# W-Ted/F3D-Gaus

Hardware: AMD Instinct MI355X
Metric: rendered views/sec at 256x256 (N Gaussians, K cams) (higher is better)
Workload: dtype f32; 1 GPU; C2: 1 image/GPU, 196608 Gaussians (sigma0=0.01), 120-view orbit @256x256, GOF forward raster only; timed region = render + 8-bit RGB frames copied to pinned host memory; compositing arithmetic: fast = error-free float32 pairs for the float64 island + hardware exp/rcp/rsq; every channel within 1e-4 of the oracle (RGB <= 3e-7), EXCEPT that the distortion channel (values 1e-7..1e-5 from cancelling fl; gaussians=196608, views=120, resolution=256, tile_cull=1, views_per_call=120, render_mode=fast, channels=all, parallelism=single GPU

## Files before the change

### f3d-gaus_amd/csrc/f3dg_binning.hip

```cpp
#include "f3dg_common.h"

namespace {

typedef unsigned long long u64;
typedef unsigned int u32;

__global__ void __launch_bounds__(F3DG_BLOCK)
scan_reduce_kernel(const u32* __restrict__ in, u64 n, u32* __restrict__ block_sums)
{
    __shared__ u32 wsum[F3DG_BLOCK / 64];
    const u64 base = (u64)blockIdx.x * F3DG_SCAN_CHUNK;
    u32 s = 0;
#pragma unroll
    for (int i = 0; i < F3DG_SCAN_ITEMS; i++) {
        const u64 k = base + (u64)i * F3DG_BLOCK + threadIdx.x;
        if (k < n) s += in[k];
    }
#pragma unroll
    for (int off = 32; off > 0; off >>= 1) s += __shfl_down(s, off, 64);
    if ((threadIdx.x & 63) == 0) wsum[threadIdx.x >> 6] = s;
    __syncthreads();
    if (threadIdx.x == 0) block_sums[blockIdx.x] = wsum[0] + wsum[1] + wsum[2] + wsum[3];
}

__global__ void __launch_bounds__(1024)
scan_blocksums_kernel(u32* __restrict__ block_sums, u32 nblocks, F3dgHeader* __restrict__ hdr)
{
    __shared__ u32 wtot[16];
    __shared__ u32 carry_s;
    __shared__ u64 carry64_s, wtot64[16];
    if (threadIdx.x == 0) { carry_s = 0; carry64_s = 0; }
    __syncthreads();
    const int lane = threadIdx.x & 63, wave = threadIdx.x >> 6;
    for (u32 start = 0; start < nblocks; start += 1024) {
        const u32 i = start + threadIdx.x;
        const u32 v = i < nblocks ? block_sums[i] : 0;
        u32 x = v;
#pragma unroll
        for (int off = 1; off < 64; off <<= 1) {
            const u32 y = __shfl_up(x, off, 64);
            if (lane >= off) x += y;
        }
        if (lane == 63) wtot[wave] = x;
        unsigned long long v64 = v;
#pragma unroll
        for (int off = 32; off > 0; off >>= 1) v64 += __shfl_down(v64, off, 64);
        if (lane == 0) wtot64[wave] = v64;
        __syncthreads();
        u32 wave_off = 0;
        for (int w = 0; w < wave; w++) wave_off += wtot[w];
        const u32 carry = carry_s;
        if (i < nblocks) block_sums[i] = carry + wave_off + x - v;
        __syncthreads();
        if (threadIdx.x == 1023) {
            carry_s = carry + wave_off + x;
            u64 t = 0;
            for (int w = 0; w < 16; w++) t += wtot64[w];
            carry64_s += t;
        }
        __syncthreads();
    }
    if (hdr && threadIdx.x == 0) {
        const u64 total = carry64_s;
        hdr->num_rendered = total > 0xFFFFFFFFull ? 0xFFFFFFFFu : (u32)total;
        hdr->overflow = total > (u64)hdr->capacity ? 1u : 0u;
    }
}

__global__ void __launch_bounds__(F3DG_BLOCK)
scan_apply_kernel(const u32* in, u32* out , u64 n, const u32* __restrict__ block_sums,
                  int exclusive)
{
    __shared__ u32 wtot[F3DG_BLOCK / 64];
    const u64 base = (u64)blockIdx.x * F3DG_SCAN_CHUNK + (u64)threadIdx.x * F3DG_SCAN_ITEMS;
    u32 v[F3DG_SCAN_ITEMS];
    u32 s = 0;
    if (base + F3DG_SCAN_ITEMS <= n) {
#pragma unroll
        for (int i = 0; i < F3DG_SCAN_ITEMS / 4; i++) {
            const uint4 w = reinterpret_cast<const uint4*>(in + base)[i];
            v[4 * i] = w.x; v[4 * i + 1] = w.y; v[4 * i + 2] = w.z; v[4 * i + 3] = w.w;
        }
    } else {
#pragma unroll
        for (int i = 0; i < F3DG_SCAN_ITEMS; i++) v[i] = (base + i < n) ? in[base + i] : 0;
    }
#pragma unroll
    for (int i = 0; i < F3DG_SCAN_ITEMS; i++) s += v[i];
    const int lane = threadIdx.x & 63, wave = threadIdx.x >> 6;
    u32 x = s;
#pragma unroll
    for (int off = 1; off < 64; off <<= 1) {
        const u32 y = __shfl_up(x, off, 64);
        if (lane >= off) x += y;
    }
    if (lane == 63) wtot[wave] = x;
    __syncthreads();
    u32 run = block_sums[blockIdx.x] + x - s;
    for (int w = 0; w < wave; w++) run += wtot[w];
    u32 o[F3DG_SCAN_ITEMS];
#pragma unroll
    for (int i = 0; i < F3DG_SCAN_ITEMS; i++) {
        const u32 before = run;
        run += v[i];
        o[i] = exclusive ? before : run;
    }
    if (base + F3DG_SCAN_ITEMS <= n) {
#pragma unroll
        for (int i = 0; i < F3DG_SCAN_ITEMS / 4; i++)
            reinterpret_cast<uint4*>(out + base)[i] = make_uint4(o[4 * i], o[4 * i + 1], o[4 * i + 2], o[4 * i + 3]);
    } else {
#pragma unroll
        for (int i = 0; i < F3DG_SCAN_ITEMS; i++)
            if (base + i < n) out[base + i] = o[i];
    }
}


struct SegChunk {
    u64 seg_base;
    u64 obase;
    u32 n;
    u32 cps;
    u32 c;
    u32 seg;
};

struct SegTable {
    const u32* vstart;
    const u32* bglob;
    const u32* xprefix;
    u32 xstride;
    u32 V;
};

struct ShiftDigit {
    int shift;
    u32 mask = 255u;
    __device__ __forceinline__ u32 operator()(u32 k) const { return (k >> shift) & mask; }
};
struct CompactDigit {
    u32 kbase;
    __device__ __forceinline__ u32 operator()(u32 k) const { const u32 d = (k - kbase) >> 16; return d < 255u ? d : 255u; }
};

template <typename K, typename DIGIT, bool MINMAX = false>
__device__ __forceinline__ void hist_chunk(const K* __restrict__ keys, const SegChunk& ck, const DIGIT digit, u32* __restrict__ hist,
                                           u32 (*h)[256], u32* __restrict__ minmax = nullptr)
{
    u32 kmin = 0xFFFFFFFFu, kmax = 0u;
#pragma unroll
    for (int w = 0; w < F3DG_BLOCK / 64; w++) h[w][threadIdx.x] = 0;
    __syncthreads();
    u32* hw = h[threadIdx.x >> 6];
    constexpr int VEC = 16 / (int)sizeof(K);
    typedef K __attribute__((ext_vector_type(VEC))) KV;
    const u64 base = (u64)ck.c * F3DG_SORT_CHUNK;
    const u64 g0 = ck.seg_base + base;
    const u64 g1 = ck.seg_base + ((u64)ck.n - base < (u64)F3DG_SORT_CHUNK ? (u64)ck.n : base + F3DG_SORT_CHUNK);
    for (u64 a = (g0 & ~(u64)(VEC - 1)) + (u64)threadIdx.x * VEC; a < g1; a += (u64)F3DG_BLOCK * VEC) {
        const KV w = *reinterpret_cast<const KV*>(keys + a);
#pragma unroll
        for (int q = 0; q < VEC; q++) {
            if (a + q >= g0 && a + q < g1) {
                const u32 key = (u32)w[q];
                atomicAdd(&hw[digit(key)], 1u);
                if (MINMAX && key != 0xFFFFFFFFu) { kmin = key < kmin ? key : kmin; kmax = key > kmax ? key : kmax; }
            }
        }
    }
    __shared__ u32 wmm[2][F3DG_BLOCK / 64];
    if (MINMAX) {
#pragma unroll
        for (int off = 32; off > 0; off >>= 1) {
            const u32 a = __shfl_down(kmin, off, 64), b = __shfl_down(kmax, off, 64);
            kmin = a < kmin ? a : kmin; kmax = b > kmax ? b : kmax;
        }
        if ((threadIdx.x & 63) == 0) { wmm[0][threadIdx.x >> 6] = kmin; wmm[1][threadIdx.x >> 6] = kmax; }
    }
    __syncthreads();
    if (MINMAX && threadIdx.x == 0) {
        u32 a = wmm[0][0], b = wmm[1][0];
#pragma unroll
        for (int w = 1; w < F3DG_BLOCK / 64; w++) { a = wmm[0][w] < a ? wmm[0][w] : a; b = wmm[1][w] > b ? wmm[1][w] : b; }
        minmax[0] = a; minmax[1] = b;
    }
    hist[ck.obase + (u64)threadIdx.x * ck.cps + ck.c] = h[0][threadIdx.x] + h[1][threadIdx.x] + h[2][threadIdx.x] + h[3][threadIdx.x];
}

struct ScatterShared {
    u32 cnt[F3DG_BLOCK / 64][256];
    u32 lbase[256];
    u32 gdelta[256];
    u32 wtot[F3DG_BLOCK / 64];
    u32 sval[F3DG_SORT_CHUNK];
};

template <typename K, bool IOTA, typename DIGIT>
__device__ __forceinline__ void scatter_chunk(const K* __restrict__ keys_in, const u32* __restrict__ vals_in, K* __restrict__ keys_out,
                                              u32* __restrict__ vals_out, const SegChunk& ck, const DIGIT digit,
                                              const u32* __restrict__ offsets , ScatterShared& sh, K* skey)
{
    const u32 n = ck.n;
    const u64 block_base = (u64)ck.c * F3DG_SORT_CHUNK;
    const u32 in_block = (u32)((n - block_base) < (u64)F3DG_SORT_CHUNK ? (n - block_base) : (u64)F3DG_SORT_CHUNK);
    const int lane = threadIdx.x & 63, wave = threadIdx.x >> 6;
#pragma unroll
    for (int w = 0; w < F3DG_BLOCK / 64; w++) sh.cnt[w][threadIdx.x] = 0;
    __syncthreads();

    const u64 wave_base = block_base + (u64)wave * (64 * F3DG_SORT_ITEMS);
    u32 key[F3DG_SORT_ITEMS];
    u32 val[F3DG_SORT_ITEMS];
    u32 rank[F3DG_SORT_ITEMS];
    const u64 lane_lt = ((u64)1 << lane) - 1;
#pragma unroll
    for (int r = 0; r < F3DG_SORT_ITEMS; r++) {
        const u64 i = wave_base + (u64)r * 64 + lane;
        const bool valid = i < n;
        key[r] = valid ? (u32)keys_in[ck.seg_base + i] : 0u;
        val[r] = IOTA ? (u32)i : (valid ? vals_in[ck.seg_base + i] : 0u);
    }
#pragma unroll
    for (int r = 0; r < F3DG_SORT_ITEMS; r++) {
        const u64 i = wave_base + (u64)r * 64 + lane;
        const bool valid = i < n;
        const u32 d = digit(key[r]);
        u64 diff = 0;
#pragma unroll
        for (int b = 0; b < 8; b++) {
            const u32 own = (u32)((int)(d << (31 - b)) >> 31);
            const u64 bal = __ballot(own != 0u);
            diff |= bal ^ (((u64)own << 32) | own);
        }
        const u64 same = __ballot(valid) & ~diff;
        const u32 below = (u32)__popcll(same & lane_lt);
        const u32 prev = sh.cnt[wave][d];
        rank[r] = prev + below;
        __builtin_amdgcn_wave_barrier();
        if (valid && below == 0) sh.cnt[wave][d] = prev + (u32)__popcll(same);
        __builtin_amdgcn_wave_barrier();
    }
    __syncthreads();
    {
        const u32 d = threadIdx.x;
        const u32 c0 = sh.cnt[0][d], c1 = sh.cnt[1][d], c2 = sh.cnt[2][d], c3 = sh.cnt[3][d];
        const u32 tot = c0 + c1 + c2 + c3;
        u32 x = tot;
#pragma unroll
        for (int off = 1; off < 64; off <<= 1) {
            const u32 y = __shfl_up(x, off, 64);
            if (lane >= off) x += y;
        }
        if (lane == 63) sh.wtot[wave] = x;
        __syncthreads();
        u32 excl = x - tot;
        for (int w = 0; w < wave; w++) excl += sh.wtot[w];
        sh.lbase[d] = excl;
        sh.gdelta[d] = offsets[ck.obase + (u64)d * ck.cps + ck.c] - excl;
        sh.cnt[0][d] = excl;
        sh.cnt[1][d] = excl + c0;
        sh.cnt[2][d] = excl + c0 + c1;
        sh.cnt[3][d] = excl + c0 + c1 + c2;
    }
    __syncthreads();
#pragma unroll
    for (int r = 0; r < F3DG_SORT_ITEMS; r++) {
        const u64 i = wave_base + (u64)r * 64 + lane;
        if (i < n) {
            const u32 d = digit(key[r]);
            const u32 slot = sh.cnt[wave][d] + rank[r];
            skey[slot] = (K)key[r];
            sh.sval[slot] = val[r];
        }
    }
    __syncthreads();
    for (u32 slot = threadIdx.x; slot < in_block; slot += F3DG_BLOCK) {
        const K k = skey[slot];
        const u32 d = digit((u32)k);
        const u32 pos = sh.gdelta[d] + slot;
        if (keys_out) keys_out[pos] = k;
        vals_out[pos] = sh.sval[slot];
    }
}

__device__ __forceinline__ SegChunk fixed_chunk(u32 seg_len, u32 cps)
{
    u32 seg, c;
    f3dg_xcd_map(blockIdx.x, gridDim.x / cps, cps, seg, c);
    SegChunk ck;
    ck.seg_base = (u64)seg * seg_len; ck.obase = (u64)seg * 256u * cps; ck.n = seg_len; ck.cps = cps; ck.c = c; ck.seg = seg;
    return ck;
}

__device__ __forceinline__ bool gsort_compact(const u32* __restrict__ minmax, u32 view, u32& kbase)
{
    const u32 kmin = minmax[2 * view], kmax = minmax[2 * view + 1];
    kbase = kmin & 0xFFFF0000u;
    return kmin <= kmax && ((kmax - kbase) >> 24) == 0u;
}

template <int PASS>
__global__ void __launch_bounds__(F3DG_BLOCK)
gsort_hist_kernel(const u32* __restrict__ keys, u32 seg_len, u32 cps, u32* __restrict__ hist, const u32* __restrict__ minmax,
                  u32* __restrict__ chunk_minmax)
{
    __shared__ u32 h[F3DG_BLOCK / 64][256];
    const SegChunk ck = fixed_chunk(seg_len, cps);
    if constexpr (PASS == 0) {
        hist_chunk<u32, ShiftDigit>(keys, ck, ShiftDigit{0}, hist, h);
    } else if constexpr (PASS == 1) {
        hist_chunk<u32, ShiftDigit, true>(keys, ck, ShiftDigit{8}, hist, h, chunk_minmax + 2 * ((size_t)ck.seg * cps + ck.c));
    } else {
        u32 kbase;
        const bool compact = gsort_compact(minmax, ck.seg, kbase);
        if (!compact) {
            hist_chunk<u32, ShiftDigit>(keys, ck, ShiftDigit{8 * PASS}, hist, h);
        } else if constexpr (PASS == 2) {
            hist_chunk<u32, CompactDigit>(keys, ck, CompactDigit{kbase}, hist, h);
        } else {
            const u64 base = (u64)ck.c * F3DG_SORT_CHUNK;
            const u32 in_chunk = (u32)((ck.n - base) < (u64)F3DG_SORT_CHUNK ? (ck.n - base) : (u64)F3DG_SORT_CHUNK);
            hist[ck.obase + (u64)threadIdx.x * ck.cps + ck.c] = threadIdx.x == 0 ? in_chunk : 0u;
        }
    }
}

__global__ void __launch_bounds__(1024)
gsort_scan_kernel(u32 n_per_seg , u32 seg_len, u32* __restrict__ hist)
{
    __shared__ u32 wtot[16];
    __shared__ u32 carry_s;
    u32* h = hist + (size_t)blockIdx.x * n_per_seg;
    const u32 lane = threadIdx.x & 63u, wave = threadIdx.x >> 6;
    if (threadIdx.x == 0) carry_s = blockIdx.x * seg_len;
    __syncthreads();
    for (u32 base = 0; base < n_per_seg; base += 4096u) {
        const u32 i = base + 4u * threadIdx.x;
        uint4 v = make_uint4(0u, 0u, 0u, 0u);
        if (i < n_per_seg) v = *reinterpret_cast<const uint4*>(h + i);
        const u32 tot = v.x + v.y + v.z + v.w;
        u32 x = tot;
#pragma unroll
        for (int off = 1; off < 64; off <<= 1) {
            const u32 y = __shfl_up(x, off, 64);
            if (lane >= (u32)off) x += y;
        }
        if (lane == 63u) wtot[wave] = x;
        __syncthreads();
        u32 before = carry_s + x - tot;
        for (u32 w = 0; w < wave; w++) before += wtot[w];
        if (i < n_per_seg)
            *reinterpret_cast<uint4*>(h + i) = make_uint4(before, before + v.x, before + v.x + v.y, before + v.x + v.y + v.z);
        __syncthreads();
        if (threadIdx.x == 1023u) carry_s = before + tot;
        __syncthreads();
    }
}

__global__ void __launch_bounds__(64)
gsort_range_kernel(u32 cps, const u32* __restrict__ chunk_minmax, u32* __restrict__ minmax)
{
    u32 kmin = 0xFFFFFFFFu, kmax = 0u;
    for (u32 c = threadIdx.x; c < cps; c += 64) {
        const u32 a = chunk_minmax[2 * ((size_t)blockIdx.x * cps + c)], b = chunk_minmax[2 * ((size_t)blockIdx.x * cps + c) + 1];
        kmin = a < kmin ? a : kmin; kmax = b > kmax ? b : kmax;
    }
#pragma unroll
    for (int off = 32; off > 0; off >>= 1) {
        const u32 a = __shfl_down(kmin, off, 64), b = __shfl_down(kmax, off, 64);
        kmin = a < kmin ? a : kmin; kmax = b > kmax ? b : kmax;
    }
    if (threadIdx.x == 0) { minmax[2 * blockIdx.x] = kmin; minmax[2 * blockIdx.x + 1] = kmax; }
}

template <int PASS>
__global__ void __launch_bounds__(F3DG_BLOCK)
gsort_scatter_kernel(const u32* __restrict__ keys_in, const u32* __restrict__ vals_in, u32* __restrict__ keys_out,
                     u32* __restrict__ vals_out, u32 seg_len, u32 cps, const u32* __restrict__ offsets, const u32* __restrict__ minmax)
{
    __shared__ ScatterShared sh;
    __shared__ u32 skey[F3DG_SORT_CHUNK];
    const SegChunk ck = fixed_chunk(seg_len, cps);
    if constexpr (PASS == 0) {
        scatter_chunk<u32, true, ShiftDigit>(keys_in, vals_in, keys_out, vals_out, ck, ShiftDigit{0}, offsets, sh, skey);
    } else if constexpr (PASS == 1) {
        scatter_chunk<u32, false, ShiftDigit>(keys_in, vals_in, keys_out, vals_out, ck, ShiftDigit{8}, offsets, sh, skey);
    } else {
        u32 kbase;
        const bool compact = gsort_compact(minmax, ck.seg, kbase);
        if (!compact)
            scatter_chunk<u32, false, ShiftDigit>(keys_in, vals_in, PASS == 3 ? (u32*)nullptr : keys_out, vals_out, ck, ShiftDigit{8 * PASS}, offsets, sh, skey);
        else if constexpr (PASS == 2)
            scatter_chunk<u32, false, CompactDigit>(keys_in, vals_in, (u32*)nullptr, vals_out, ck, CompactDigit{kbase}, offsets, sh, skey);
    }
}

__global__ void __launch_bounds__(512)
view_segments_kernel(int V, int P, const u32* __restrict__ offsets_sorted, const F3dgHeader* __restrict__ hdr, u32* __restrict__ vstart,
                     u32* __restrict__ bglob, u32* __restrict__ xprefix, u32 xstride)
{
    __shared__ u32 carry;
    __shared__ u32 wtot[8];
    const u32 lane = threadIdx.x & 63u, wave = threadIdx.x >> 6;
    const bool dead = hdr->overflow != 0;
    auto start_of = [&](u32 v) -> u32 {
        const u64 i = (u64)v * (u64)P;
        return (dead || i == 0) ? 0u : offsets_sorted[i - 1];
    };
    auto chunks_of = [&](u32 v) -> u32 {
        const u32 n = start_of(v + 1) - start_of(v);
        return (n + F3DG_SORT_CHUNK - 1) / F3DG_SORT_CHUNK;
    };
    if (threadIdx.x == 0) carry = 0;
    __syncthreads();
    for (u32 v0 = 0; v0 < (u32)V; v0 += 512) {
        const u32 v = v0 + threadIdx.x;
        const u32 c = v < (u32)V ? chunks_of(v) : 0u;
        u32 x = c;
#pragma unroll
        for (int off = 1; off < 64; off <<= 1) {
            const u32 y = __shfl_up(x, off, 64);
            if (lane >= (u32)off) x += y;
        }
        if (lane == 63) wtot[wave] = x;
        __syncthreads();
        u32 woff = carry;
        for (u32 w = 0; w < wave; w++) woff += wtot[w];
        if (v < (u32)V) { vstart[v] = start_of(v); bglob[v] = woff + x - c; }
        __syncthreads();
        if (threadIdx.x == 511) carry = woff + x;
        __syncthreads();
    }
    if (threadIdx.x == 0) { vstart[V] = start_of((u32)V); bglob[V] = carry; }
    const u32 nk = ((u32)V > wave) ? ((u32)V - wave + 7u) / 8u : 0u;
    u32 run = 0;
    for (u32 k0 = 0; k0 < nk; k0 += 64) {
        const u32 k = k0 + lane;
        const u32 c = k < nk ? chunks_of(wave + 8u * k) : 0u;
        u32 x = c;
#pragma unroll
        for (int off = 1; off < 64; off <<= 1) {
            const u32 y = __shfl_up(x, off, 64);
            if (lane >= (u32)off) x += y;
        }
        if (k < nk) xprefix[wave * xstride + k] = run + x - c;
        run += __shfl(x, 63, 64);
    }
    if (lane == 0) xprefix[wave * xstride + nk] = run;
}

__global__ void __launch_bounds__(F3DG_BLOCK)
ranges_from_offsets_kernel(u32 V, u32 T, int tile_bits, const u32* __restrict__ bglob, const u32* __restrict__ offsets,
                           const F3dgHeader* __restrict__ hdr, uint2* __restrict__ ranges)
{
    const u32 i = blockIdx.x * F3DG_BLOCK + threadIdx.x;
    if (i >= V * T) return;
    const u32 v = i / T, t = i % T;
    const u32 b0 = bglob[v], cpv = bglob[v + 1] - b0;
    uint2 r = make_uint2(0u, 0u);
    if (cpv != 0u && !hdr->overflow) {
        const u32 d = ((v << tile_bits) | t) & 255u;
        const u32 lo = offsets[256ull * b0 + (u64)d * cpv], hi = offsets[256ull * b0 + (u64)(d + 1u) * cpv];
        if (hi > lo) r = make_uint2(lo, hi);
    }
    ranges[i] = r;
}

__device__ __forceinline__ bool var_chunk(const SegTable& st, u32 f, u32& k, SegChunk& ck)
{
    const u32 x = blockIdx.x & 7u;
    const u32* xp = st.xprefix + x * st.xstride;
    const u32 nk = (st.V > x) ? (st.V - x + 7u) / 8u : 0u;
    while (k < nk && f >= xp[k + 1]) k++;
    if (k >= nk) return false;
    const u32 v = x + 8u * k;
    const u32 s0 = st.vstart[v], b0 = st.bglob[v];
    ck.seg_base = s0; ck.n = st.vstart[v + 1] - s0; ck.cps = st.bglob[v + 1] - b0; ck.obase = 256ull * b0; ck.c = f - xp[k];
    return true;
}

template <typename K>
__global__ void __launch_bounds__(F3DG_BLOCK)
radix2_hist_var_kernel(const K* __restrict__ keys, SegTable st, int shift, u32 mask, u32* __restrict__ hist)
{
    __shared__ u32 h[F3DG_BLOCK / 64][256];
    u32 k = 0;
    SegChunk ck;
    for (u32 f = blockIdx.x >> 3; var_chunk(st, f, k, ck); f += gridDim.x >> 3)
        hist_chunk<K, ShiftDigit>(keys, ck, ShiftDigit{shift, mask}, hist, h);
}

template <typename K>
__global__ void __launch_bounds__(F3DG_BLOCK)
radix2_scatter_var_kernel(const K* __restrict__ keys_in, const u32* __restrict__ vals_in, K* __restrict__ keys_out,
                          u32* __restrict__ vals_out, SegTable st, int shift, u32 mask, const u32* __restrict__ offsets)
{
    __shared__ ScatterShared sh;
    __shared__ K skey[F3DG_SORT_CHUNK];
    u32 k = 0;
    SegChunk ck;
    for (u32 f = blockIdx.x >> 3; var_chunk(st, f, k, ck); f += gridDim.x >> 3) {
        scatter_chunk<K, false, ShiftDigit>(keys_in, vals_in, keys_out, vals_out, ck, ShiftDigit{shift, mask}, offsets, sh, skey);
        __syncthreads();
    }
}

__global__ void __launch_bounds__(F3DG_BLOCK)
gsort_gather_rects_kernel(int P, u32* __restrict__ gv0, u32* __restrict__ gv1, const u32* __restrict__ minmax,
                          const uint2* __restrict__ rects, u32* __restrict__ tiles_sorted, u32* __restrict__ rx)
{
    constexpr int ITEMS = 4;
    unsigned view, chunk;
    const unsigned cpv = (unsigned)((P + F3DG_BLOCK * ITEMS - 1) / (F3DG_BLOCK * ITEMS));
    f3dg_xcd_map(blockIdx.x, gridDim.x / cpv, cpv, view, chunk);
    const size_t vb = (size_t)view * P;
    u32 kbase;
    const bool pass2 = gsort_compact(minmax, view, kbase);
    const u32* perm = pass2 ? gv1 : gv0;
    u32* ry = pass2 ? gv0 : gv1;
    const int k0 = (int)(chunk * F3DG_BLOCK * ITEMS + threadIdx.x);
    u32 id[ITEMS];
    uint2 r[ITEMS];
#pragma unroll
    for (int i = 0; i < ITEMS; i++) { const int k = k0 + i * F3DG_BLOCK; id[i] = k < P ? perm[vb + k] : 0u; }
#pragma unroll
    for (int i = 0; i < ITEMS; i++) { const int k = k0 + i * F3DG_BLOCK; r[i] = k < P ? rects[vb + id[i]] : make_uint2(0u, 0u); }
#pragma unroll
    for (int i = 0; i < ITEMS; i++) {
        const int k = k0 + i * F3DG_BLOCK;
        if (k < P) {
            tiles_sorted[vb + k] = (((r[i].x >> 16) & F3DG_RECT_COORD) - (r[i].x & F3DG_RECT_COORD)) *
                                   (((r[i].y >> 16) & F3DG_RECT_COORD) - (r[i].y & F3DG_RECT_COORD));
            rx[vb + k] = r[i].x;
            ry[vb + k] = r[i].y;
        }
    }
}

#define F3DG_DUP_CAP 3072
template <typename G>
__global__ void __launch_bounds__(F3DG_BLOCK)
duplicate_sorted_kernel(int P, int tile_bits, int grid_x, const u32* __restrict__ gv0, const u32* __restrict__ gv1,
                        const u32* __restrict__ minmax, const u32* __restrict__ rx,
                        const u32* __restrict__ offsets_sorted,
                        const F3dgHeader* __restrict__ hdr, G* __restrict__ kgrp, u32* __restrict__ vals)
{
    __shared__ G sk[F3DG_DUP_CAP];
    __shared__ u32 sv[F3DG_DUP_CAP];
    if (hdr->overflow) return;
    const int k = blockIdx.x * F3DG_BLOCK + threadIdx.x;
    const int v = blockIdx.y;
    u32 kbase;
    const bool pass2 = gsort_compact(minmax, (u32)v, kbase);
    const u32* perm = pass2 ? gv1 : gv0;
    const u32* ry = pass2 ? gv0 : gv1;
    const size_t first = (size_t)v * P + (size_t)blockIdx.x * F3DG_BLOCK;
    const int in_block = min(F3DG_BLOCK, P - (int)(blockIdx.x * F3DG_BLOCK));
    const u32 base = first == 0 ? 0u : offsets_sorted[first - 1];
    const u32 n = offsets_sorted[first + in_block - 1] - base;
    u32 off0 = 0, cnt = 0, x = 0, y = 0, g = 0;
    if (k < P) {
        const size_t pos = (size_t)v * P + k;
        x = rx[pos]; y = ry[pos];
        const u32 rminx = x & F3DG_RECT_COORD, rmaxx = (x >> 16) & F3DG_RECT_COORD, rminy = y & F3DG_RECT_COORD, rmaxy = (y >> 16) & F3DG_RECT_COORD;
        if (rmaxx > rminx && rmaxy > rminy) {
            g = perm[pos];
            off0 = ((pos == 0) ? 0 : offsets_sorted[pos - 1]) - base;
            cnt = (rmaxx - rminx) * (rmaxy - rminy);
        }
    }
    const u32 rminx = x & F3DG_RECT_COORD, rmaxx = (x >> 16) & F3DG_RECT_COORD, rminy = y & F3DG_RECT_COORD, rmaxy = (y >> 16) & F3DG_RECT_COORD;
    const u32 view_base = (u32)v << tile_bits;
    auto halves = [](u32 t, u32 tmin, u32 tmax, u32 word) -> u32 {
        u32 m = 3u;
        if (t == tmin && (word & F3DG_RECT_SKIP_LO)) m &= ~1u;
        if (t + 1u == tmax && (word & F3DG_RECT_SKIP_HI)) m &= ~2u;
        return m;
    };
    for (u32 wb = 0; wb < n; wb += (u32)F3DG_DUP_CAP) {
        const u32 lo = off0 > wb ? off0 : wb;
        const u32 hi = off0 + cnt < wb + (u32)F3DG_DUP_CAP ? off0 + cnt : wb + (u32)F3DG_DUP_CAP;
        if (lo < hi) {
            const u32 w = rmaxx - rminx, j0 = lo - off0;
            u32 ty = rminy + j0 / w, tx = rminx + j0 % w;
            u32 my = halves(ty, rminy, rmaxy, y);
            for (u32 j = lo; j < hi; j++) {
                const u32 mx = halves(tx, rminx, rmaxx, x);
                sk[j - wb] = (G)(view_base | (ty * (u32)grid_x + tx));
                sv[j - wb] = g | ((((my & 1u) ? mx : 0u) | ((my & 2u) ? mx << 2 : 0u)) << F3DG_ID_BITS);
                if (++tx == rmaxx) { tx = rminx; ty++; my = halves(ty, rminy, rmaxy, y); }
            }
        }
        __syncthreads();
        const u32 in_win = n - wb < (u32)F3DG_DUP_CAP ? n - wb : (u32)F3DG_DUP_CAP;
        for (u32 i = threadIdx.x; i < in_win; i += F3DG_BLOCK) {
            kgrp[base + wb + i] = sk[i];
            vals[base + wb + i] = sv[i];
        }
        __syncthreads();
    }
}

__global__ void __launch_bounds__(F3DG_BLOCK)
export_keys_kernel(u32 nseg, int P, int tile_bits, int T, const uint2* __restrict__ ranges, const F3dgHeader* __restrict__ hdr,
                   const u32* __restrict__ point_list, const float* __restrict__ depths, u64* __restrict__ keys_out)
{
    if (hdr->overflow) return;
    for (u32 seg = blockIdx.x; seg < nseg; seg += gridDim.x) {
        const uint2 r = ranges[seg];
        const u32 view = seg / (u32)T, tile = seg % (u32)T;
        const u64 hi = (u64)((view << tile_bits) | tile) << 32;
        for (u32 i = r.x + threadIdx.x; i < r.y; i += F3DG_BLOCK)
            keys_out[i] = hi | (u64)__float_as_uint(depths[(size_t)view * P + (point_list[i] & F3DG_ID_MASK)]);
    }
}

template <typename G>
__global__ void __launch_bounds__(F3DG_BLOCK)
group_bounds_kernel(const G* __restrict__ kgrp, const F3dgHeader* __restrict__ hdr, int tile_bits, int T, u32* __restrict__ ranges)
{
    const u32 L = hdr->overflow ? 0u : hdr->num_rendered;
    const u32 tmask = (1u << tile_bits) - 1u;
    for (u64 base = ((u64)blockIdx.x * F3DG_BLOCK + threadIdx.x) * 8u; base < L; base += (u64)gridDim.x * F3DG_BLOCK * 8u) {
        G v[8];
        if (base + 8 <= L) {
            typedef G __attribute__((ext_vector_type(8))) G8;
            const G8 w = *reinterpret_cast<const G8*>(kgrp + base);
#pragma unroll
            for (int i = 0; i < 8; i++) v[i] = w[i];
        } else {
#pragma unroll
            for (int i = 0; i < 8; i++) v[i] = base + i < L ? kgrp[base + i] : (G)0;
        }
        u32 prev = base > 0 ? (u32)kgrp[base - 1] : 0u;
        const u32 next = base + 8 < L ? (u32)kgrp[base + 8] : 0u;
#pragma unroll
        for (int i = 0; i < 8; i++) {
            const u64 idx = base + i;
            if (idx < L) {
                const u32 cur = (u32)v[i];
                const u32 nxt = i < 7 ? (u32)v[i + 1] : next;
                const u32 seg = (cur >> tile_bits) * (u32)T + (cur & tmask);
                if (idx == 0 || prev != cur) ranges[2u * seg] = (u32)idx;
                if (idx == L - 1 || nxt != cur) ranges[2u * seg + 1u] = (u32)idx + 1u;
                prev = cur;
            }
        }
    }
}

int bits_for(unsigned long long n_values)
{
    int b = 0;
    while (b < 64 && (n_values - 1) >> b) b++;
    return n_values <= 1 ? 0 : b;
}

}

int f3dg_launch_scan_inclusive(hipStream_t s, const unsigned* in, unsigned* out, unsigned long long n,
                               unsigned* tmp, unsigned tmp_elems, int exclusive, F3dgHeader* hdr_total)
{
    if (n == 0) return F3DG_OK;
    const unsigned nblocks = (unsigned)((n + F3DG_SCAN_CHUNK - 1) / F3DG_SCAN_CHUNK);
    if (nblocks > tmp_elems) return F3DG_ERR_WORKSPACE;
    F3DG_KLAUNCH(scan_reduce_kernel, dim3(nblocks), dim3(F3DG_BLOCK), 0, s, in, (u64)n, tmp);
    F3DG_KLAUNCH(scan_blocksums_kernel, dim3(1), dim3(1024), 0, s, tmp, nblocks, hdr_total);
    F3DG_KLAUNCH(scan_apply_kernel, dim3(nblocks), dim3(F3DG_BLOCK), 0, s, in, out, (u64)n, tmp, exclusive);
    F3DG_HIP_CHECK(hipGetLastError());
    return F3DG_OK;
}

int f3dg_tile_bits(int T) { return bits_for((unsigned long long)T); }


int f3dg_sort_passes(int V, int T)
{
    (void)V;
    const int bits = f3dg_tile_bits(T);
    return bits == 0 ? 0 : (bits + 7) / 8;
}

template <typename G>
static int binning_tail(hipStream_t s, int V, int P, int grid_x, int T, int tile_bits, const F3dgLayout& L, char* ws, F3dgHeader* hdr)
{
    int rc = F3DG_OK;
    const size_t VP = (size_t)V * P;
    u32* scan_tmp = reinterpret_cast<u32*>(ws + L.scan_tmp);
    u32* hist = reinterpret_cast<u32*>(ws + L.hist);
    u32* gk[2] = { reinterpret_cast<u32*>(ws + L.gsort), reinterpret_cast<u32*>(ws + L.gsort) + VP };
    u32* gv[2] = { reinterpret_cast<u32*>(ws + L.gsort) + 2 * VP, reinterpret_cast<u32*>(ws + L.gsort) + 3 * VP };
    G* kgrp[2] = { reinterpret_cast<G*>(ws + L.keys[0]), reinterpret_cast<G*>(ws + L.keys[1]) };
    u32* vals[2] = { reinterpret_cast<u32*>(ws + L.vals[0]), reinterpret_cast<u32*>(ws + L.vals[1]) };
    const dim3 pgrid((P + F3DG_BLOCK - 1) / F3DG_BLOCK, V);

    const u32 cps = (u32)((P + F3DG_SORT_CHUNK - 1) / F3DG_SORT_CHUNK);
    const u32 gblocks = (u32)V * cps;
    u32* minmax = reinterpret_cast<u32*>(ws + L.segtab) + L.segtab_minmax;
    u32* chunk_minmax = minmax + 2 * (size_t)V;
    const bool view_scan = cps <= 64;
#define F3DG_GSORT_PASS(PASS, IN, OUT)                                                                                                     \
    F3DG_KLAUNCH((gsort_hist_kernel<PASS>), dim3(gblocks), dim3(F3DG_BLOCK), 0, s, gk[IN], (u32)P, cps, hist, minmax, chunk_minmax); \
    if (view_scan)                                                                                                                         \
        F3DG_KLAUNCH(gsort_scan_kernel, dim3(V), dim3(1024), 0, s, 256u * cps, (u32)P, hist);                                       \
    else {                                                                                                                                 \
        rc = f3dg_launch_scan_inclusive(s, hist, hist, (unsigned long long)256 * gblocks, scan_tmp, L.scan_tmp_elems, 1, nullptr);        \
        if (rc != F3DG_OK) return rc;                                                                                                      \
    }                                                                                                                                      \
    F3DG_KLAUNCH((gsort_scatter_kernel<PASS>), dim3(gblocks), dim3(F3DG_BLOCK), 0, s, gk[IN], gv[IN], gk[OUT], gv[OUT], (u32)P, cps, hist, minmax)
    F3DG_GSORT_PASS(0, 0, 1);
    F3DG_GSORT_PASS(1, 1, 0);
    F3DG_KLAUNCH(gsort_range_kernel, dim3(V), dim3(64), 0, s, cps, chunk_minmax, minmax);
    F3DG_GSORT_PASS(2, 0, 1);
    F3DG_GSORT_PASS(3, 1, 0);
#undef F3DG_GSORT_PASS
    u32* offsets_sorted = gk[1];
    u32* rx = gk[0];

    F3DG_KLAUNCH(gsort_gather_rects_kernel, dim3((unsigned)V * (unsigned)((P + 4 * F3DG_BLOCK - 1) / (4 * F3DG_BLOCK))), dim3(F3DG_BLOCK), 0, s, P, gv[0], gv[1], minmax,
                           reinterpret_cast<const uint2*>(ws + L.rects), offsets_sorted, rx);
    rc = f3dg_launch_scan_inclusive(s, offsets_sorted, offsets_sorted, (unsigned long long)VP, scan_tmp, L.scan_tmp_elems, 0, hdr);
    if (rc != F3DG_OK) return rc;
    const int passes = f3dg_sort_passes(V, T);
    int src = passes & 1;
    F3DG_KLAUNCH((duplicate_sorted_kernel<G>), pgrid, dim3(F3DG_BLOCK), 0, s, P, tile_bits, grid_x, gv[0], gv[1], minmax, rx, offsets_sorted, hdr,
                       kgrp[src], vals[src]);

    if (passes > 0) {
        SegTable st;
        u32* segtab = reinterpret_cast<u32*>(ws + L.segtab);
        const u32 xstride = (u32)V / 8u + 2u;
        st.vstart = segtab; st.bglob = segtab + (V + 1); st.xprefix = segtab + 2 * (V + 1); st.xstride = xstride; st.V = (u32)V;
        F3DG_KLAUNCH(view_segments_kernel, dim3(1), dim3(512), 0, s, V, P, offsets_sorted, hdr, segtab, segtab + (V + 1),
                           segtab + 2 * (V + 1), xstride);
        const size_t nbmax = (size_t)L.sort_blocks + (size_t)V;
        const u32 per_xcd = (u32)((nbmax + 7) / 8 < 160 ? (nbmax + 7) / 8 : 160);
        const u32 per_xcd_h = (u32)((nbmax + 7) / 8 < 512 ? (nbmax + 7) / 8 : 512);
        const int split = passes == 2 ? (tile_bits + 1) / 2 : 8;
        for (int p = 0; p < passes; p++) {
            const int shift = split * p;
            const u32 mask = passes == 2 ? (1u << (p == 0 ? split : tile_bits - split)) - 1u : 255u;
            F3DG_HIP_CHECK(hipMemsetAsync(hist, 0, sizeof(u32) * 256 * nbmax, s));
            F3DG_KLAUNCH((radix2_hist_var_kernel<G>), dim3(8 * per_xcd_h), dim3(F3DG_BLOCK), 0, s, kgrp[src], st, shift, mask, hist);
            rc = f3dg_launch_scan_inclusive(s, hist, hist, (unsigned long long)256 * nbmax, scan_tmp, L.scan_tmp_elems, 1, nullptr);
            if (rc != F3DG_OK) return rc;
            F3DG_KLAUNCH((radix2_scatter_var_kernel<G>), dim3(8 * per_xcd), dim3(F3DG_BLOCK), 0, s, kgrp[src], vals[src],
                               passes == 1 ? (G*)nullptr : kgrp[src ^ 1], vals[src ^ 1], st, shift, mask, hist);
            src ^= 1;
        }
        if (passes == 1) {
            const u32 nseg = (u32)V * (u32)T;
            F3DG_KLAUNCH(ranges_from_offsets_kernel, dim3((nseg + F3DG_BLOCK - 1) / F3DG_BLOCK), dim3(F3DG_BLOCK), 0, s, (u32)V, (u32)T, tile_bits,
                               segtab + (V + 1), hist, hdr, reinterpret_cast<uint2*>(ws + L.ranges));
            F3DG_HIP_CHECK(hipGetLastError());
            return F3DG_OK;
        }
    }
    F3DG_HIP_CHECK(hipMemsetAsync(ws + L.ranges, 0, sizeof(uint2) * (size_t)V * T, s));
    F3DG_KLAUNCH((group_bounds_kernel<G>), dim3(2048), dim3(F3DG_BLOCK), 0, s, kgrp[0], hdr, tile_bits, T, reinterpret_cast<u32*>(ws + L.ranges));
    F3DG_HIP_CHECK(hipGetLastError());
    return F3DG_OK;
}

int f3dg_launch_binning(hipStream_t s, int V, int P, int W, int H, const F3dgLayout& L, char* ws, int export_offsets)
{
    const int grid_x = (W + F3DG_TILE - 1) / F3DG_TILE, grid_y = (H + F3DG_TILE - 1) / F3DG_TILE;
    const int T = grid_x * grid_y;
    const int tile_bits = f3dg_tile_bits(T);
    F3dgHeader* hdr = reinterpret_cast<F3dgHeader*>(ws + L.header);

    int rc = F3DG_OK;
    if (export_offsets) {
        rc = f3dg_launch_scan_inclusive(s, reinterpret_cast<const u32*>(ws + L.tiles), reinterpret_cast<u32*>(ws + L.offsets),
                                        (unsigned long long)V * P, reinterpret_cast<u32*>(ws + L.scan_tmp), L.scan_tmp_elems, 0, nullptr);
        if (rc != F3DG_OK) return rc;
    }
    const bool small = (((unsigned long long)(V > 0 ? V - 1 : 0) << tile_bits) | ((1ull << tile_bits) - 1ull)) <= 0xFFFFull;
    rc = small ? binning_tail<unsigned short>(s, V, P, grid_x, T, tile_bits, L, ws, hdr)
               : binning_tail<u32>(s, V, P, grid_x, T, tile_bits, L, ws, hdr);
    if (rc != F3DG_OK) return rc;
    F3DG_HIP_CHECK(hipGetLastError());
    return F3DG_OK;
}

int f3dg_launch_export_keys(hipStream_t s, int V, int P, int W, int H, const F3dgLayout& L, char* ws)
{
    const int grid_x = (W + F3DG_TILE - 1) / F3DG_TILE, grid_y = (H + F3DG_TILE - 1) / F3DG_TILE;
    const int T = grid_x * grid_y;
    const u32 nseg = (u32)V * (u32)T;
    const u32 rg = nseg < 65535u * 4u ? nseg : 65535u * 4u;
    F3DG_KLAUNCH(export_keys_kernel, dim3(rg), dim3(F3DG_BLOCK), 0, s, nseg, P, f3dg_tile_bits(T), T,
                       reinterpret_cast<const uint2*>(ws + L.ranges), reinterpret_cast<const F3dgHeader*>(ws + L.header),
                       reinterpret_cast<const u32*>(ws + L.vals[0]), reinterpret_cast<const float*>(ws + L.depths),
                       reinterpret_cast<u64*>(ws + L.keys[0]));
    F3DG_HIP_CHECK(hipGetLastError());
    return F3DG_OK;
}
```

Baseline: 31170 views/s.

## Replace global per-Gaussian offset scan with block sums and per-view segmented scans

Instead of writing per-Gaussian tile counts and running a full device-wide inclusive scan over V*P entries, the gather kernel now emits per-block sums. These are scanned per view, and the duplicate kernel recomputes local offsets with an in-block wave scan. The radix histogram memset plus global scan is replaced by a per-view in-place tile scan kernel that also produces tile ranges, which removes the separate ranges kernel. This cuts global memory traffic and kernel launches. In exchange, overflow detection and num_rendered are now computed in view_segments_kernel, and the histogram memset is dropped, so the histogram kernel must fully overwrite its buffer.

```diff
diff --git a/f3d-gaus_amd/csrc/f3dg_binning.hip b/f3d-gaus_amd/csrc/f3dg_binning.hip
--- a/f3d-gaus_amd/csrc/f3dg_binning.hip
+++ b/f3d-gaus_amd/csrc/f3dg_binning.hip
@@ -326,20 +326,24 @@
     }
 }
 
-__global__ void __launch_bounds__(1024)
-gsort_scan_kernel(u32 n_per_seg , u32 seg_len, u32* __restrict__ hist)
+template <int VECS>
+__device__ __forceinline__ void scan_in_place_1024(u32* h, u32 n, u32 start)
 {
     __shared__ u32 wtot[16];
     __shared__ u32 carry_s;
-    u32* h = hist + (size_t)blockIdx.x * n_per_seg;
     const u32 lane = threadIdx.x & 63u, wave = threadIdx.x >> 6;
-    if (threadIdx.x == 0) carry_s = blockIdx.x * seg_len;
-    __syncthreads();
-    for (u32 base = 0; base < n_per_seg; base += 4096u) {
-        const u32 i = base + 4u * threadIdx.x;
-        uint4 v = make_uint4(0u, 0u, 0u, 0u);
-        if (i < n_per_seg) v = *reinterpret_cast<const uint4*>(h + i);
-        const u32 tot = v.x + v.y + v.z + v.w;
+    if (threadIdx.x == 0) carry_s = start;
+    __syncthreads();
+    for (u32 base = 0; base < n; base += 4096u * VECS) {
+        const u32 i = base + 4u * VECS * threadIdx.x;
+        uint4 v[VECS];
+        u32 tot = 0;
+#pragma unroll
+        for (int q = 0; q < VECS; q++) {
+            v[q] = make_uint4(0u, 0u, 0u, 0u);
+            if (i + 4u * q < n) v[q] = *reinterpret_cast<const uint4*>(h + i + 4u * q);
+            tot += v[q].x + v[q].y + v[q].z + v[q].w;
+        }
         u32 x = tot;
 #pragma unroll
         for (int off = 1; off < 64; off <<= 1) {
@@ -350,12 +354,23 @@
         __syncthreads();
         u32 before = carry_s + x - tot;
         for (u32 w = 0; w < wave; w++) before += wtot[w];
-        if (i < n_per_seg)
-            *reinterpret_cast<uint4*>(h + i) = make_uint4(before, before + v.x, before + v.x + v.y, before + v.x + v.y + v.z);
+        u32 run = before;
+#pragma unroll
+        for (int q = 0; q < VECS; q++) {
+            if (i + 4u * q < n)
+                *reinterpret_cast<uint4*>(h + i + 4u * q) = make_uint4(run, run + v[q].x, run + v[q].x + v[q].y, run + v[q].x + v[q].y + v[q].z);
+            run += v[q].x + v[q].y + v[q].z + v[q].w;
+        }
         __syncthreads();
         if (threadIdx.x == 1023u) carry_s = before + tot;
         __syncthreads();
     }
+}
+
+__global__ void __launch_bounds__(1024)
+gsort_scan_kernel(u32 n_per_seg , u32 seg_len, u32* __restrict__ hist)
+{
+    scan_in_place_1024<1>(hist + (size_t)blockIdx.x * n_per_seg, n_per_seg, blockIdx.x * seg_len);
 }
 
 __global__ void __launch_bounds__(64)
@@ -396,43 +411,101 @@
     }
 }
 
+
+__device__ __forceinline__ u32 rect_tiles(u32 x, u32 y)
+{
+    const u32 rminx = x & F3DG_RECT_COORD, rmaxx = (x >> 16) & F3DG_RECT_COORD, rminy = y & F3DG_RECT_COORD, rmaxy = (y >> 16) & F3DG_RECT_COORD;
+    return (rmaxx > rminx && rmaxy > rminy) ? (rmaxx - rminx) * (rmaxy - rminy) : 0u;
+}
+
+__global__ void __launch_bounds__(1024)
+view_blocks_scan_kernel(u32 nb, u32* __restrict__ block_sums, u64* __restrict__ view_total)
+{
+    __shared__ u32 wtot[16];
+    __shared__ u32 carry_s;
+    __shared__ u64 carry64_s, wtot64[16];
+    u32* h = block_sums + (size_t)blockIdx.x * nb;
+    if (threadIdx.x == 0) { carry_s = 0; carry64_s = 0; }
+    __syncthreads();
+    const int lane = threadIdx.x & 63, wave = threadIdx.x >> 6;
+    for (u32 start = 0; start < nb; start += 1024) {
+        const u32 i = start + threadIdx.x;
+        const u32 v = i < nb ? h[i] : 0;
+        u32 x = v;
+#pragma unroll
+        for (int off = 1; off < 64; off <<= 1) {
+            const u32 y = __shfl_up(x, off, 64);
+            if (lane >= off) x += y;
+        }
+        if (lane == 63) wtot[wave] = x;
+        u64 v64 = v;
+#pragma unroll
+        for (int off = 32; off > 0; off >>= 1) v64 += __shfl_down(v64, off, 64);
+        if (lane == 0) wtot64[wave] = v64;
+        __syncthreads();
+        u32 wave_off = 0;
+        for (int w = 0; w < wave; w++) wave_off += wtot[w];
+        const u32 carry = carry_s;
+        if (i < nb) h[i] = carry + wave_off + x - v;
+        __syncthreads();
+        if (threadIdx.x == 1023) {
+            carry_s = carry + wave_off + x;
+            u64 t = 0;
+            for (int w = 0; w < 16; w++) t += wtot64[w];
+            carry64_s += t;
+        }
+        __syncthreads();
+    }
+    if (threadIdx.x == 0) view_total[blockIdx.x] = carry64_s;
+}
+
 __global__ void __launch_bounds__(512)
-view_segments_kernel(int V, int P, const u32* __restrict__ offsets_sorted, const F3dgHeader* __restrict__ hdr, u32* __restrict__ vstart,
+view_segments_kernel(int V, const u64* __restrict__ view_total, F3dgHeader* __restrict__ hdr, u32* __restrict__ vstart,
                      u32* __restrict__ bglob, u32* __restrict__ xprefix, u32 xstride)
 {
-    __shared__ u32 carry;
-    __shared__ u32 wtot[8];
+    __shared__ u32 carry, ncarry, dead_s;
+    __shared__ u32 wtot[8], ntot[8];
+    __shared__ u64 wtot64[8];
     const u32 lane = threadIdx.x & 63u, wave = threadIdx.x >> 6;
-    const bool dead = hdr->overflow != 0;
-    auto start_of = [&](u32 v) -> u32 {
-        const u64 i = (u64)v * (u64)P;
-        return (dead || i == 0) ? 0u : offsets_sorted[i - 1];
-    };
-    auto chunks_of = [&](u32 v) -> u32 {
-        const u32 n = start_of(v + 1) - start_of(v);
-        return (n + F3DG_SORT_CHUNK - 1) / F3DG_SORT_CHUNK;
-    };
-    if (threadIdx.x == 0) carry = 0;
-    __syncthreads();
+    u64 t = 0;
+    for (u32 v = threadIdx.x; v < (u32)V; v += 512) t += view_total[v];
+#pragma unroll
+    for (int off = 32; off > 0; off >>= 1) t += __shfl_down(t, off, 64);
+    if (lane == 0) wtot64[wave] = t;
+    __syncthreads();
+    if (threadIdx.x == 0) {
+        u64 total = 0;
+        for (int w = 0; w < 8; w++) total += wtot64[w];
+        const u32 over = total > (u64)hdr->capacity ? 1u : 0u;
+        hdr->num_rendered = total > 0xFFFFFFFFull ? 0xFFFFFFFFu : (u32)total;
+        hdr->overflow = over;
+        dead_s = over;
+        carry = 0; ncarry = 0;
+    }
+    __syncthreads();
+    const bool dead = dead_s != 0;
+    auto count_of = [&](u32 v) -> u32 { return dead ? 0u : (u32)view_total[v]; };
+    auto chunks_of = [&](u32 v) -> u32 { return (count_of(v) + F3DG_SORT_CHUNK - 1) / F3DG_SORT_CHUNK; };
     for (u32 v0 = 0; v0 < (u32)V; v0 += 512) {
         const u32 v = v0 + threadIdx.x;
-        const u32 c = v < (u32)V ? chunks_of(v) : 0u;
-        u32 x = c;
+        const u32 n = v < (u32)V ? count_of(v) : 0u;
+        const u32 c = (n + F3DG_SORT_CHUNK - 1) / F3DG_SORT_CHUNK;
+        u32 x = c, xn = n;
 #pragma unroll
         for (int off = 1; off < 64; off <<= 1) {
-            const u32 y = __shfl_up(x, off, 64);
-            if (lane >= (u32)off) x += y;
-        }
-        if (lane == 63) wtot[wave] = x;
-        __syncthreads();
-        u32 woff = carry;
-        for (u32 w = 0; w < wave; w++) woff += wtot[w];
-        if (v < (u32)V) { vstart[v] = start_of(v); bglob[v] = woff + x - c; }
-        __syncthreads();
-        if (threadIdx.x == 511) carry = woff + x;
-        __syncthreads();
-    }
-    if (threadIdx.x == 0) { vstart[V] = start_of((u32)V); bglob[V] = carry; }
+            const u32 y = __shfl_up(x, off, 64), yn = __shfl_up(xn, off, 64);
+            if (lane >= (u32)off) { x += y; xn += yn; }
+        }
+        if (lane == 63) { wtot[wave] = x; ntot[wave] = xn; }
+        __syncthreads();
+        u32 woff = carry, noff = ncarry;
+        for (u32 w = 0; w < wave; w++) { woff += wtot[w]; noff += ntot[w]; }
+        if (v < (u32)V) { vstart[v] = noff + xn - n; bglob[v] = woff + x - c; }
+        __syncthreads();
+        if (threadIdx.x == 511) { carry = woff + x; ncarry = noff + xn; }
+        __syncthreads();
+    }
+    if (threadIdx.x == 0) { vstart[V] = ncarry; bglob[V] = carry; }
     const u32 nk = ((u32)V > wave) ? ((u32)V - wave + 7u) / 8u : 0u;
     u32 run = 0;
     for (u32 k0 = 0; k0 < nk; k0 += 64) {
@@ -450,21 +523,26 @@
     if (lane == 0) xprefix[wave * xstride + nk] = run;
 }
 
-__global__ void __launch_bounds__(F3DG_BLOCK)
-ranges_from_offsets_kernel(u32 V, u32 T, int tile_bits, const u32* __restrict__ bglob, const u32* __restrict__ offsets,
-                           const F3dgHeader* __restrict__ hdr, uint2* __restrict__ ranges)
-{
-    const u32 i = blockIdx.x * F3DG_BLOCK + threadIdx.x;
-    if (i >= V * T) return;
-    const u32 v = i / T, t = i % T;
-    const u32 b0 = bglob[v], cpv = bglob[v + 1] - b0;
-    uint2 r = make_uint2(0u, 0u);
-    if (cpv != 0u && !hdr->overflow) {
-        const u32 d = ((v << tile_bits) | t) & 255u;
-        const u32 lo = offsets[256ull * b0 + (u64)d * cpv], hi = offsets[256ull * b0 + (u64)(d + 1u) * cpv];
-        if (hi > lo) r = make_uint2(lo, hi);
-    }
-    ranges[i] = r;
+__global__ void __launch_bounds__(1024)
+tile_scan_kernel(SegTable st, u32* hist, u32 T, int tile_bits, const F3dgHeader* __restrict__ hdr, uint2* __restrict__ ranges)
+{
+    const u32 v = blockIdx.x;
+    const u32 b0 = st.bglob[v], cpv = st.bglob[v + 1] - b0;
+    u32* h = hist + 256ull * b0;
+    scan_in_place_1024<4>(h, 256u * cpv, st.vstart[v]);
+    if (!ranges) return;
+    __syncthreads();
+    const bool live = cpv != 0u && !hdr->overflow;
+    const u32 vend = st.vstart[v + 1];
+    for (u32 t = threadIdx.x; t < T; t += 1024u) {
+        uint2 r = make_uint2(0u, 0u);
+        if (live) {
+            const u32 d = ((v << tile_bits) | t) & 255u;
+            const u32 lo = h[(size_t)d * cpv], hi = d == 255u ? vend : h[(size_t)(d + 1u) * cpv];
+            if (hi > lo) r = make_uint2(lo, hi);
+        }
+        ranges[(size_t)v * T + t] = r;
+    }
 }
 
 __device__ __forceinline__ bool var_chunk(const SegTable& st, u32 f, u32& k, SegChunk& ck)
@@ -508,9 +586,10 @@
 
 __global__ void __launch_bounds__(F3DG_BLOCK)
 gsort_gather_rects_kernel(int P, u32* __restrict__ gv0, u32* __restrict__ gv1, const u32* __restrict__ minmax,
-                          const uint2* __restrict__ rects, u32* __restrict__ tiles_sorted, u32* __restrict__ rx)
+                          const uint2* __restrict__ rects, u32* __restrict__ block_sums, u32* __restrict__ rx)
 {
     constexpr int ITEMS = 4;
+    __shared__ u32 wsum[ITEMS][F3DG_BLOCK / 64];
     unsigned view, chunk;
     const unsigned cpv = (unsigned)((P + F3DG_BLOCK * ITEMS - 1) / (F3DG_BLOCK * ITEMS));
     f3dg_xcd_map(blockIdx.x, gridDim.x / cpv, cpv, view, chunk);
@@ -529,13 +608,19 @@
 #pragma unroll
     for (int i = 0; i < ITEMS; i++) {
         const int k = k0 + i * F3DG_BLOCK;
+        u32 n = 0;
         if (k < P) {
-            tiles_sorted[vb + k] = (((r[i].x >> 16) & F3DG_RECT_COORD) - (r[i].x & F3DG_RECT_COORD)) *
-                                   (((r[i].y >> 16) & F3DG_RECT_COORD) - (r[i].y & F3DG_RECT_COORD));
+            n = rect_tiles(r[i].x, r[i].y);
             rx[vb + k] = r[i].x;
             ry[vb + k] = r[i].y;
         }
-    }
+#pragma unroll
+        for (int off = 32; off > 0; off >>= 1) n += __shfl_down(n, off, 64);
+        if ((threadIdx.x & 63) == 0) wsum[i][threadIdx.x >> 6] = n;
+    }
+    __syncthreads();
+    const unsigned nb = (unsigned)((P + F3DG_BLOCK - 1) / F3DG_BLOCK), b = chunk * ITEMS + threadIdx.x;
+    if (threadIdx.x < ITEMS && b < nb) block_sums[(size_t)view * nb + b] = wsum[threadIdx.x][0] + wsum[threadIdx.x][1] + wsum[threadIdx.x][2] + wsum[threadIdx.x][3];
 }
 
 #define F3DG_DUP_CAP 3072
@@ -543,11 +628,12 @@
 __global__ void __launch_bounds__(F3DG_BLOCK)
 duplicate_sorted_kernel(int P, int tile_bits, int grid_x, const u32* __restrict__ gv0, const u32* __restrict__ gv1,
                         const u32* __restrict__ minmax, const u32* __restrict__ rx,
-                        const u32* __restrict__ offsets_sorted,
+                        const u32* __restrict__ block_offsets, const u32* __restrict__ vstart,
                         const F3dgHeader* __restrict__ hdr, G* __restrict__ kgrp, u32* __restrict__ vals)
 {
     __shared__ G sk[F3DG_DUP_CAP];
     __shared__ u32 sv[F3DG_DUP_CAP];
+    __shared__ u32 wtot[F3DG_BLOCK / 64];
     if (hdr->overflow) return;
     const int k = blockIdx.x * F3DG_BLOCK + threadIdx.x;
     const int v = blockIdx.y;
@@ -555,21 +641,25 @@
     const bool pass2 = gsort_compact(minmax, (u32)v, kbase);
     const u32* perm = pass2 ? gv1 : gv0;
     const u32* ry = pass2 ? gv0 : gv1;
-    const size_t first = (size_t)v * P + (size_t)blockIdx.x * F3DG_BLOCK;
-    const int in_block = min(F3DG_BLOCK, P - (int)(blockIdx.x * F3DG_BLOCK));
-    const u32 base = first == 0 ? 0u : offsets_sorted[first - 1];
-    const u32 n = offsets_sorted[first + in_block - 1] - base;
-    u32 off0 = 0, cnt = 0, x = 0, y = 0, g = 0;
+    const u32 base = vstart[v] + block_offsets[(size_t)v * gridDim.x + blockIdx.x];
+    u32 cnt = 0, x = 0, y = 0, g = 0;
     if (k < P) {
         const size_t pos = (size_t)v * P + k;
         x = rx[pos]; y = ry[pos];
-        const u32 rminx = x & F3DG_RECT_COORD, rmaxx = (x >> 16) & F3DG_RECT_COORD, rminy = y & F3DG_RECT_COORD, rmaxy = (y >> 16) & F3DG_RECT_COORD;
-        if (rmaxx > rminx && rmaxy > rminy) {
-            g = perm[pos];
-            off0 = ((pos == 0) ? 0 : offsets_sorted[pos - 1]) - base;
-            cnt = (rmaxx - rminx) * (rmaxy - rminy);
-        }
-    }
+        cnt = rect_tiles(x, y);
+        if (cnt) g = perm[pos];
+    }
+    u32 off0 = cnt;
+#pragma unroll
+    for (int off = 1; off < 64; off <<= 1) {
+        const u32 up = __shfl_up(off0, off, 64);
+        if ((threadIdx.x & 63) >= off) off0 += up;
+    }
+    if ((threadIdx.x & 63) == 63) wtot[threadIdx.x >> 6] = off0;
+    __syncthreads();
+    off0 -= cnt;
+    for (int w = 0; w < (int)(threadIdx.x >> 6); w++) off0 += wtot[w];
+    const u32 n = wtot[0] + wtot[1] + wtot[2] + wtot[3];
     const u32 rminx = x & F3DG_RECT_COORD, rmaxx = (x >> 16) & F3DG_RECT_COORD, rminy = y & F3DG_RECT_COORD, rmaxy = (y >> 16) & F3DG_RECT_COORD;
     const u32 view_base = (u32)v << tile_bits;
     auto halves = [](u32 t, u32 tmin, u32 tmax, u32 word) -> u32 {
@@ -715,25 +805,25 @@
     F3DG_GSORT_PASS(2, 0, 1);
     F3DG_GSORT_PASS(3, 1, 0);
 #undef F3DG_GSORT_PASS
-    u32* offsets_sorted = gk[1];
+    const u32 nb = pgrid.x;
+    u32* block_sums = gk[1];
     u32* rx = gk[0];
+    u64* view_total = reinterpret_cast<u64*>(hist);
 
     F3DG_KLAUNCH(gsort_gather_rects_kernel, dim3((unsigned)V * (unsigned)((P + 4 * F3DG_BLOCK - 1) / (4 * F3DG_BLOCK))), dim3(F3DG_BLOCK), 0, s, P, gv[0], gv[1], minmax,
-                           reinterpret_cast<const uint2*>(ws + L.rects), offsets_sorted, rx);
-    rc = f3dg_launch_scan_inclusive(s, offsets_sorted, offsets_sorted, (unsigned long long)VP, scan_tmp, L.scan_tmp_elems, 0, hdr);
-    if (rc != F3DG_OK) return rc;
+                           reinterpret_cast<const uint2*>(ws + L.rects), block_sums, rx);
+    F3DG_KLAUNCH(view_blocks_scan_kernel, dim3(V), dim3(1024), 0, s, nb, block_sums, view_total);
+    SegTable st;
+    u32* segtab = reinterpret_cast<u32*>(ws + L.segtab);
+    const u32 xstride = (u32)V / 8u + 2u;
+    st.vstart = segtab; st.bglob = segtab + (V + 1); st.xprefix = segtab + 2 * (V + 1); st.xstride = xstride; st.V = (u32)V;
+    F3DG_KLAUNCH(view_segments_kernel, dim3(1), dim3(512), 0, s, V, view_total, hdr, segtab, segtab + (V + 1), segtab + 2 * (V + 1), xstride);
     const int passes = f3dg_sort_passes(V, T);
     int src = passes & 1;
-    F3DG_KLAUNCH((duplicate_sorted_kernel<G>), pgrid, dim3(F3DG_BLOCK), 0, s, P, tile_bits, grid_x, gv[0], gv[1], minmax, rx, offsets_sorted, hdr,
+    F3DG_KLAUNCH((duplicate_sorted_kernel<G>), pgrid, dim3(F3DG_BLOCK), 0, s, P, tile_bits, grid_x, gv[0], gv[1], minmax, rx, block_sums, segtab, hdr,
                        kgrp[src], vals[src]);
 
     if (passes > 0) {
-        SegTable st;
-        u32* segtab = reinterpret_cast<u32*>(ws + L.segtab);
-        const u32 xstride = (u32)V / 8u + 2u;
-        st.vstart = segtab; st.bglob = segtab + (V + 1); st.xprefix = segtab + 2 * (V + 1); st.xstride = xstride; st.V = (u32)V;
-        F3DG_KLAUNCH(view_segments_kernel, dim3(1), dim3(512), 0, s, V, P, offsets_sorted, hdr, segtab, segtab + (V + 1),
-                           segtab + 2 * (V + 1), xstride);
         const size_t nbmax = (size_t)L.sort_blocks + (size_t)V;
         const u32 per_xcd = (u32)((nbmax + 7) / 8 < 160 ? (nbmax + 7) / 8 : 160);
         const u32 per_xcd_h = (u32)((nbmax + 7) / 8 < 512 ? (nbmax + 7) / 8 : 512);
@@ -741,18 +831,14 @@
         for (int p = 0; p < passes; p++) {
             const int shift = split * p;
             const u32 mask = passes == 2 ? (1u << (p == 0 ? split : tile_bits - split)) - 1u : 255u;
-            F3DG_HIP_CHECK(hipMemsetAsync(hist, 0, sizeof(u32) * 256 * nbmax, s));
             F3DG_KLAUNCH((radix2_hist_var_kernel<G>), dim3(8 * per_xcd_h), dim3(F3DG_BLOCK), 0, s, kgrp[src], st, shift, mask, hist);
-            rc = f3dg_launch_scan_inclusive(s, hist, hist, (unsigned long long)256 * nbmax, scan_tmp, L.scan_tmp_elems, 1, nullptr);
-            if (rc != F3DG_OK) return rc;
+            F3DG_KLAUNCH(tile_scan_kernel, dim3(V), dim3(1024), 0, s, st, hist, (u32)T, tile_bits, hdr,
+                               passes == 1 ? reinterpret_cast<uint2*>(ws + L.ranges) : (uint2*)nullptr);
             F3DG_KLAUNCH((radix2_scatter_var_kernel<G>), dim3(8 * per_xcd), dim3(F3DG_BLOCK), 0, s, kgrp[src], vals[src],
                                passes == 1 ? (G*)nullptr : kgrp[src ^ 1], vals[src ^ 1], st, shift, mask, hist);
             src ^= 1;
         }
         if (passes == 1) {
-            const u32 nseg = (u32)V * (u32)T;
-            F3DG_KLAUNCH(ranges_from_offsets_kernel, dim3((nseg + F3DG_BLOCK - 1) / F3DG_BLOCK), dim3(F3DG_BLOCK), 0, s, (u32)V, (u32)T, tile_bits,
-                               segtab + (V + 1), hist, hdr, reinterpret_cast<uint2*>(ws + L.ranges));
             F3DG_HIP_CHECK(hipGetLastError());
             return F3DG_OK;
         }
```

New measurement: 31090 views/s. No clear change (-0.2%).
